# google-research/weatherbench2

Hardware: AMD Instinct MI355X
Metric: grid-point-evals/sec (721x1440x13) (higher is better)
Workload: dtype f32 (elementwise) + f64 (sums); 1 GPU; BASELINE configs[1]: 721x1440x13 f32, deterministic MSE+RMSE+MAE+Bias+ACC, 13 predefined slice regions, running init-time mean; pool_units=48, regions=13, rows_per_chunk=32, step=one wb2_det_suite_step call (K1 + K2 + time accumulate), parallelism=init-time shards x1, 1 all-reduce of [sum,count], launcher=single process

## Files before the change

### weatherbench2_amd/csrc/energy_score.hip

```cpp
#include "ensemble_kernels.hpp"

namespace wb2 {
namespace {

constexpr int kEnergyWaves = 8;
#ifndef WB2_ENERGY_B
#define WB2_ENERGY_B 8
#endif
#ifndef WB2_ENERGY_ROWS
#define WB2_ENERGY_ROWS 4
#endif

template <typename T, int B, bool SKIPNA, bool WF>
__global__ void __launch_bounds__(kEnergyWaves* kWave)
    energy_partials_kernel(const EnsParams p, const int n_block) {
  constexpr int KQ = 2 * B, K = SKIPNA ? 2 * KQ : KQ, NWF = WF ? 2 : 1;
  const int lane = threadIdx.x & (kWave - 1);
  const int wave = __builtin_amdgcn_readfirstlane(threadIdx.x / kWave);
  const unsigned bx = blockIdx.x;
  const long long o = (long long)blockIdx.z * gridDim.y + blockIdx.y;
  const unsigned rest = bx / (unsigned)p.n_chunk;
  const int chunk = (int)(((long long)(bx - rest * (unsigned)p.n_chunk) +
                           (WB2_ROTATE_CHUNKS ? o : 0)) % p.n_chunk);
  const int tile = (int)(rest % (unsigned)p.n_ctile);
// ... 13 lines not shown
  const int colc = active ? col0 : p.n_col - 1;

  double acc[NWF][1][K];
#pragma unroll
  for (int w = 0; w < NWF; ++w)
#pragma unroll
    for (int k = 0; k < K; ++k) acc[w][0][k] = 0.0;

  const long long slab_elems = (long long)p.n_row * p.n_col;
  const T* xrow0 = static_cast<const T*>(p.ens) + es * slab_elems +
                   (long long)m0 * p.member_stride + (long long)row0 * p.n_col;
  const int lane_bytes = colc * (int)sizeof(T);
  const T* tb = static_cast<const T*>(p.truth) + ts * slab_elems +
                (long long)row0 * p.n_col + colc;
  const double* wfp =
      WF ? p.wfield + (long long)row0 * p.n_col + colc : nullptr;
  constexpr int U = WB2_ENERGY_ROWS;
  auto rows = [&](const int r, auto count_tag) {
    constexpr int N = decltype(count_tag)::value;
    T x[N][B + 1], t[N];
    double wr[N], wf[N];
#pragma unroll
    for (int u = 0; u < N; ++u) {
      const long long off = (long long)(r + u) * p.n_col;
      const T* xrow = xrow0 + off;
#pragma unroll
      for (int j = 0; j <= B; ++j)
        x[u][j] = member_load<T, true>(xrow + j * p.member_stride, lane_bytes,
                                       j < nload ? 0x7fffffff : 0);
      t[u] = __builtin_nontemporal_load(tb + off);
      wr[u] = p.w_row[row0 + r + u];
      wf[u] = 1.0;
      if constexpr (WF) wf[u] = wfp[off];
    }
#pragma unroll
    for (int u = 0; u < N; ++u) {
      const bool inside = !WF || wf[u] > 0.0;
      const double w2 = (WF && inside) ? wr[u] * wf[u] : 0.0;
      auto add = [&](int k, T q, bool live) {
        if (!live) return;
        double v = (double)q, c = 1.0;
        if constexpr (SKIPNA) {
          const bool ok = !is_nan(q);
          v = ok ? v : 0.0;
          c = ok ? 1.0 : 0.0;
        }
        acc[0][0][k] = __builtin_fma(wr[u], v, acc[0][0][k]);
        if constexpr (SKIPNA)
          acc[0][0][KQ + k] = __builtin_fma(wr[u], c, acc[0][0][KQ + k]);
        if constexpr (WF) {
          acc[1][0][k] = __builtin_fma(w2, inside ? v : 0.0, acc[1][0][k]);
          if constexpr (SKIPNA)
            acc[1][0][KQ + k] =
                __builtin_fma(w2, inside ? c : 0.0, acc[1][0][KQ + k]);
        }
      };
#pragma unroll
      for (int j = 0; j < B; ++j) {
        const T d = x[u][j] - t[u];
        add(j, d * d, j < nm);
        const T e = x[u][j] - x[u][j + 1];
        add(B + j, e * e, j < np);
      }
    }
  };
  int r = 0;
#pragma clang loop unroll(disable)
  for (; r + U <= nrow; r += U) rows(r, std::integral_constant<int, U>{});
#pragma clang loop unroll(disable)
  for (; r < nrow; ++r) rows(r, std::integral_constant<int, 1>{});
  if (p.w_col) {
    const double wc = p.w_col[colc];
#pragma unroll
    for (int w = 0; w < NWF; ++w)
#pragma unroll
      for (int k = 0; k < K; ++k) acc[w][0][k] *= wc;
  }
  if (!active) {
#pragma unroll
    for (int w = 0; w < NWF; ++w)
#pragma unroll
      for (int k = 0; k < K; ++k) acc[w][0][k] = 0.0;
  }
  fold_tile_to_segs<NWF, 1, K>(
      acc, lane, tile, col0, col0, p.n_col, p.seg_col0, p.seg_eoff, p.n_seg,
      p.n_ts,
      p.partials + ((o * n_block + block) * p.n_chunk + chunk) *
                       (long long)(NWF * p.n_ts * K));
}

constexpr int kEnergyMaxMembers = 1024;
__global__ void __launch_bounds__(kWave)
    energy_finalize_kernel(const double* __restrict__ means, int block,
                           int n_block, int n_member, int skipna, int n_region,
                           long long n_outer, double* __restrict__ out) {
  __shared__ double root[2][kEnergyMaxMembers];
  const long long idx = blockIdx.x;
  const int lane = threadIdx.x;
  const int r = (int)(idx / n_outer);
  const long long o = idx - (long long)r * n_outer;
  const long long n_virtual = n_outer * n_block;
  const long long row = (long long)n_region * n_virtual;
  const double* base = means + (long long)r * n_virtual + o * n_block;
  for (int m = lane; m < n_member; m += kWave) {
    root[0][m] = sqrt(base[(long long)(m % block) * row + m / block]);
    if (m + 1 < n_member)
      root[1][m] = sqrt(base[(long long)(block + m % block) * row + m / block]);
  }
  __syncthreads();
  if (lane != 0) return;
  auto member_mean = [&](const double* v, int count) {
    double s = 0.0, n = 0.0;
    for (int m = 0; m < count; ++m) {
      const bool keep = !(skipna && is_nan(v[m]));
      s += keep ? v[m] : 0.0;
      n += keep ? 1.0 : 0.0;
    }
    return s / n;
  };
  const double skill = member_mean(root[0], n_member);
  const double spread = n_member == 1 ? 0.0 : member_mean(root[1], n_member - 1);
  const long long plane = (long long)n_region * n_outer;
  out[idx] = skill - 0.5 * spread;
  out[plane + idx] = spread;
  out[2 * plane + idx] = skill;
}

template <typename T, int B>
int launch_energy(const EnsParams& p, int n_block, bool skipna, bool wf,
                  hipStream_t stream) {
  const int n_bgrp = (n_block + kEnergyWaves - 1) / kEnergyWaves;
  const int waves = n_block < kEnergyWaves ? n_block : kEnergyWaves;
  const long long gy = p.n_outer < 32768 ? p.n_outer : 32768;
  const long long gz = (p.n_outer + gy - 1) / gy;
  const dim3 grid((unsigned)(p.n_chunk * p.n_ctile * n_bgrp), (unsigned)gy,
                  (unsigned)gz);
  const dim3 blockdim(waves * kWave);
#define WB2_L(S, W)                                                       \
  hipLaunchKernelGGL((energy_partials_kernel<T, B, S, W>), grid, blockdim, 0, \
                     stream, p, n_block)
  if (skipna) {
    if (wf) WB2_L(true, true); else WB2_L(true, false);
  } else {
    if (wf) WB2_L(false, true); else WB2_L(false, false);
  }
#undef WB2_L
  WB2_HIP_OK(hipGetLastError());
  return 0;
}

int energy_block(bool skipna, bool wf) {
  return (skipna && wf) ? 4 : WB2_ENERGY_B;
}

}
}

extern "C" {

int wb2_energy_layout(int32_t n_member, int skipna, int has_wfield,
                      int32_t* block, int32_t* n_block, int32_t* n_slot) {
  using namespace wb2;
  WB2_REQUIRE(n_member >= 1, "n_member=%d", n_member);
  WB2_REQUIRE(block && n_block && n_slot, "null pointer argument");
  const int b = energy_block(skipna != 0, has_wfield != 0);
  *block = b;
  *n_block = (n_member + b - 1) / b;
// ... 89 lines not shown
```

### weatherbench2_amd/csrc/reduce_common.hpp

```cpp
#pragma once

#include "common.hpp"

#include <cstdint>

#ifndef WB2_ROTATE_CHUNKS
#define WB2_ROTATE_CHUNKS 1
#endif

namespace wb2 {

int combine_slots(int mode, int skipna, int k_slots, const double* partials,
                  int64_t n_outer, int32_t n_chunk, int32_t nwf, int32_t n_seg,
                  const int32_t* seg_eoff, int32_t n_ts,
                  const int32_t* band_chunk0, int32_t n_band,
                  const double* coef_band, const double* coef_seg,
                  const int32_t* region_wf, const double* region_wsum,
                  int32_t n_region, double* sums, double* metrics,
                  void* stream);

__device__ __forceinline__ void swap_halves32(double& a, double& b) {
  const unsigned long long ua = __builtin_bit_cast(unsigned long long, a);
  const unsigned long long ub = __builtin_bit_cast(unsigned long long, b);
  const auto lo = __builtin_amdgcn_permlane32_swap(
// ... 7 lines not shown
  const unsigned long long ua = __builtin_bit_cast(unsigned long long, a);
  const unsigned long long ub = __builtin_bit_cast(unsigned long long, b);
  const auto lo = __builtin_amdgcn_permlane16_swap(
      (unsigned)ua, (unsigned)ub, false, false);
  const auto hi = __builtin_amdgcn_permlane16_swap(
      (unsigned)(ua >> 32), (unsigned)(ub >> 32), false, false);
  a = __builtin_bit_cast(double, ((unsigned long long)hi[0] << 32) | lo[0]);
  b = __builtin_bit_cast(double, ((unsigned long long)hi[1] << 32) | lo[1]);
}

template <int CTRL>
__device__ __forceinline__ double dpp_move(double x) {
  const unsigned long long u = __builtin_bit_cast(unsigned long long, x);
  const unsigned lo = (unsigned)__builtin_amdgcn_update_dpp(
      0, (int)(unsigned)u, CTRL, 0xf, 0xf, false);
  const unsigned hi = (unsigned)__builtin_amdgcn_update_dpp(
      0, (int)(unsigned)(u >> 32), CTRL, 0xf, 0xf, false);
  return __builtin_bit_cast(double, ((unsigned long long)hi << 32) | lo);
}

template <int OFF>
__device__ __forceinline__ double allsum_low_bits(double v) {
  static_assert(OFF >= 1 && OFF <= 32, "lane bit");

  if constexpr (OFF >= 32) v += __shfl_xor(v, 32, kWave);
  if constexpr (OFF >= 16) v += __shfl_xor(v, 16, kWave);
  if constexpr (OFF >= 8) v += dpp_move<0x128>(v);
  if constexpr (OFF >= 4) {
    const unsigned long long u = __builtin_bit_cast(unsigned long long, v);
    const unsigned lo = (unsigned)__builtin_amdgcn_ds_swizzle((int)(unsigned)u,
                                                              0x101F);
    const unsigned hi = (unsigned)__builtin_amdgcn_ds_swizzle(
        (int)(unsigned)(u >> 32), 0x101F);
    v += __builtin_bit_cast(double, ((unsigned long long)hi << 32) | lo);
  }
  if constexpr (OFF >= 2) v += dpp_move<0x4E>(v);
  v += dpp_move<0xB1>(v);
  return v;
}

template <int N, int OFF, int NV>
__device__ __forceinline__ void wave_sum_many_step(double (&v)[NV], int lane,
                                                   int& slot, int& real,
                                                   bool& writer) {
  if constexpr (OFF == 0) {
    return;
  } else if constexpr (N == 1) {
    v[0] = allsum_low_bits<OFF>(v[0]);
    writer = writer && (lane & (2 * OFF - 1)) == 0;
  } else {
    constexpr int H = (N + 1) / 2;
    const bool up = (lane & OFF) != 0;
#pragma unroll
    for (int i = 0; i < H; ++i) {
      double lo = v[i];
      double hi = (H + i < N) ? v[H + i] : 0.0;
      if constexpr (OFF == 32) {
        swap_halves32(lo, hi);
        v[i] = lo + hi;
      } else if constexpr (OFF == 16) {
        swap_halves16(lo, hi);
        v[i] = lo + hi;
      } else {
        const double keep = up ? hi : lo, send = up ? lo : hi;
        v[i] = keep + __shfl_xor(send, OFF, kWave);
      }
    }
    slot += up ? H : 0;
    real = up ? (real > H ? real - H : 0) : (real < H ? real : H);
    wave_sum_many_step<H, OFF / 2, NV>(v, lane, slot, real, writer);
  }
}

template <int N>
__device__ __forceinline__ void wave_sum_many(double (&v)[N], int lane,
                                              int& slot, bool& writes) {
  int real = N;
  bool writer = true;
  slot = 0;
  wave_sum_many_step<N, 32, N>(v, lane, slot, real, writer);
  writes = writer && real > 0;
}

template <int NWF, int VEC, int K>
__device__ __forceinline__ void fold_tile_to_segs(
    const double (&acc)[NWF][VEC][K], int lane, int tile, int col0, int own0,
    int n_col, const int* __restrict__ seg_col0, const int* __restrict__ seg_eoff,
    int n_seg, int n_ts, double* __restrict__ out) {
  constexpr int TILE = kWave * VEC;
  const int tile_c0 = tile * TILE;
  const int tile_c1 = min(tile_c0 + TILE, n_col);
  int s_lo = 0;
  while (seg_col0[s_lo + 1] <= tile_c0) ++s_lo;
  int s_hi = s_lo;
  while (s_hi + 1 < n_seg && seg_col0[s_hi + 1] < tile_c1) ++s_hi;
  for (int s = s_lo; s <= s_hi; ++s) {
    const int c0 = seg_col0[s], c1 = seg_col0[s + 1];
    double v[NWF * K];
#pragma unroll
    for (int w = 0; w < NWF; ++w) {
#pragma unroll
      for (int k = 0; k < K; ++k) v[w * K + k] = 0.0;
#pragma unroll
      for (int e = 0; e < VEC; ++e) {
        const bool in_seg = (col0 + e >= max(c0, own0)) && (col0 + e < c1);
#pragma unroll
        for (int k = 0; k < K; ++k)
          v[w * K + k] += in_seg ? acc[w][e][k] : 0.0;
      }
    }
    int slot;
    bool writes;
    wave_sum_many<NWF * K>(v, lane, slot, writes);
    const int e = seg_eoff[s] + tile - c0 / TILE;
    if (writes) {
      const int w = slot / K, k = slot - w * K;
      out[((long long)w * n_ts + e) * K + k] = v[0];
    }
  }
}

}
```

### weatherbench2_amd/csrc/stream_reduce.hip

```cpp

#include "common.hpp"
#include "trace.hpp"
#include "reduce_common.hpp"
#include "gauss_math.hpp"
#include "wb2hip.h"

#include <atomic>
#include <type_traits>

namespace wb2 {
namespace {

constexpr int kMaxIn = 4;

struct StreamParams {
  const void* in[kMaxIn];
  const long long* slab[kMaxIn];
  const double* w_row;
  const double* w_col;
  const void* wfield;
  const double* aux;
  double scalar;
  const int* chunk_row0;
  const int* chunk_nrow;
// ... 193 lines not shown
        x[k] = v[k];
      }
    }
  } else if constexpr (MODE == WB2_MODE_GAUSS) {
    const T mean = in[0], sd = in[1], y = in[2];
    const T nd = (mean - y) / sd;
    const double z = (double)nd;
    double cdf, pdf;
    far = normal_cdf_pdf<ERFCX_FAR>(z, erfcx_lds, cdf, pdf);
    const double crps =
        (double)sd * (z * (2.0 * cdf - 1.0) + 2.0 * pdf - 0.56418958354775628695);
    const T var = sd * sd;
    if constexpr (SKIPNA) {
      const bool okc = !is_nan(crps), okv = !is_nan(var);
      x[0] = okc ? crps : 0.0;
      x[1] = okv ? (double)var : 0.0;
      x[2] = okc ? 1.0 : 0.0;
      x[3] = okv ? 1.0 : 0.0;
    } else {
      x[0] = crps;
      x[1] = (double)var;
    }
  } else {
    T q[PointOps<MODE>::NQ];
    PointOps<MODE>::template elementwise<T>(in, q);
    PointOps<MODE>::template slots<SKIPNA, T>(q, x);
  }
  return far;
}

#ifndef WB2_U_ROWS
#define WB2_U_ROWS 2
#endif
#ifndef WB2_U_ROWS_NARROW
#define WB2_U_ROWS_NARROW 8
#endif
#ifndef WB2_F32_VEC
#define WB2_F32_VEC 4
#endif
#ifndef WB2_F32_VEC_HEAVY
#define WB2_F32_VEC_HEAVY 4
#endif
#ifndef WB2_NT_LOADS
#define WB2_NT_LOADS 1
#endif
#ifndef WB2_GAUSS_GROUP
#define WB2_GAUSS_GROUP 2
#endif
#ifndef WB2_PACK_PAIRS
#define WB2_PACK_PAIRS 1
#endif

#if WB2_NT_LOADS
#define WB2_LOAD(ptr) __builtin_nontemporal_load(ptr)
#else
#define WB2_LOAD(ptr) (*(ptr))
#endif

#define WB2_GLOBAL __attribute__((address_space(1)))

template <typename T, int VEC>
__device__ __forceinline__ void load_vec(const WB2_GLOBAL T* p, T (&v)[VEC]) {
  if constexpr (VEC == 1) {
    v[0] = WB2_LOAD(p);
  } else {
    typedef T V0 __attribute__((ext_vector_type(VEC)));
    typedef V0 V __attribute__((aligned(sizeof(T))));
    const V0 x = WB2_LOAD(reinterpret_cast<const WB2_GLOBAL V*>(p));
#pragma unroll
    for (int e = 0; e < VEC; ++e) v[e] = x[e];
  }
}

template <int VEC, typename FT>
__device__ __forceinline__ void load_wf(const WB2_GLOBAL FT* p,
                                        double (&v)[VEC]) {
  typedef FT V0 __attribute__((ext_vector_type(VEC)));
  typedef V0 V __attribute__((aligned(sizeof(FT))));
  const V0 x = *reinterpret_cast<const WB2_GLOBAL V*>(p);
#pragma unroll
  for (int e = 0; e < VEC; ++e) v[e] = (double)x[e];
}

template <typename T, int VEC, int MODE, bool SKIPNA, bool WF,
          bool SG = false, typename FT = double>
__global__ void __launch_bounds__(512)
    stream_partials_kernel(const StreamParams p) {
  using M = ModeTraits<MODE, SKIPNA>;
  constexpr int NIN = M::NIN, K = M::K, NWF = WF ? 2 : 1;
  constexpr int U = (sizeof(T) * VEC >= 16)
                        ? (NIN >= 4 ? WB2_U_ROWS / 2 : WB2_U_ROWS)
                        : (sizeof(T) * VEC == 8 ? 2 * WB2_U_ROWS
                                                : WB2_U_ROWS_NARROW);
  constexpr int TILE = kWave * VEC;

  const int lane = threadIdx.x & (kWave - 1);
  const int wave = __builtin_amdgcn_readfirstlane(threadIdx.x / kWave);
  const int nwave = blockDim.x / kWave;
  constexpr bool SLAB_FASTEST = WF || MODE == WB2_MODE_SEEPS;
  const unsigned bx = SLAB_FASTEST ? blockIdx.y : blockIdx.x;
  const unsigned tblk = bx / (unsigned)p.n_chunk;
  const long long o =
      SLAB_FASTEST ? (long long)blockIdx.z * gridDim.x + blockIdx.x
                   : (long long)blockIdx.z * gridDim.y + blockIdx.y;
  int chunk = (int)(bx - tblk * (unsigned)p.n_chunk);
  if (!SLAB_FASTEST && WB2_ROTATE_CHUNKS)
    chunk = (int)(((long long)chunk + o) % p.n_chunk);
  const int tile = (int)tblk * nwave + wave;

  const int row0 = p.chunk_row0[chunk];
  const int nrow = p.chunk_nrow[chunk];
  long long slab_idx[NIN];
#pragma unroll
  for (int i = 0; i < NIN; ++i) {
    const long long* tab =
        p.slab[i] ? p.slab[i] : reinterpret_cast<const long long*>(p.chunk_row0);
    const long long v = tab[(p.slab[i] && o < p.n_outer) ? o : 0];
    slab_idx[i] = p.slab[i] ? v : o;
  }
  const int col0 = tile * TILE + lane * VEC;
  const bool active = tile < p.n_ctile && col0 < p.n_col;
  const int colb = (VEC > 1 && col0 + VEC > p.n_col) ? p.n_col - VEC : col0;
  [[maybe_unused]] const double* erfcx_lds = nullptr;
  if constexpr (MODE == WB2_MODE_GAUSS || MODE == WB2_MODE_GAUSS_THR) {
    __shared__ __attribute__((aligned(16))) double erfcx_table[kErfcxDoubles];
    load_erfcx_table(erfcx_table);
    erfcx_lds = erfcx_table;
  }
  if (nrow <= 0 || tile >= p.n_ctile || o >= p.n_outer) return;

  double acc[NWF][VEC][K];
#pragma unroll
  for (int w = 0; w < NWF; ++w)
#pragma unroll
    for (int e = 0; e < VEC; ++e)
#pragma unroll
      for (int k = 0; k < K; ++k) acc[w][e][k] = 0.0;

  if (active) {
    const T* base[NIN];
#pragma unroll
    for (int i = 0; i < NIN; ++i)
      base[i] = reinterpret_cast<const T*>(
                    static_cast<const char*>(p.in[i]) +
                    slab_idx[i] * p.slab_step_bytes) +
                (long long)row0 * p.n_col;
    const FT* wfp =
        WF ? static_cast<const FT*>(p.wfield) + (long long)row0 * p.n_col
           : nullptr;
    const double* wrp = p.w_row + row0;
    unsigned lane_off = (unsigned)colb * (unsigned)sizeof(T);
    unsigned lane_off_wf = (unsigned)colb * (unsigned)sizeof(FT);
    auto at = [&](const T* row) {
      if constexpr (SG) {
        unsigned long long rp = reinterpret_cast<unsigned long long>(row);
        asm volatile("" : "+s"(rp));
        return reinterpret_cast<const WB2_GLOBAL T*>(
            reinterpret_cast<const WB2_GLOBAL char*>(rp) + lane_off);
      } else {
        return reinterpret_cast<const WB2_GLOBAL T*>(
            reinterpret_cast<unsigned long long>(row + colb));
      }
    };
    auto at_wf = [&](const FT* row) {
      if constexpr (SG) {
        unsigned long long rp = reinterpret_cast<unsigned long long>(row);
        asm volatile("" : "+s"(rp));
        return reinterpret_cast<const WB2_GLOBAL FT*>(
            reinterpret_cast<const WB2_GLOBAL char*>(rp) + lane_off_wf);
      } else {
        return reinterpret_cast<const WB2_GLOBAL FT*>(
            reinterpret_cast<unsigned long long>(row + colb));
      }
    };
    auto pin_offsets = [&]() {
      if constexpr (SG) {
        asm volatile("" : "+v"(lane_off));
        if constexpr (WF) asm volatile("" : "+v"(lane_off_wf));
      }
    };

    auto accumulate = [&](int e, const double (&x)[K], double wfe, double wr) {
#pragma unroll
      for (int k = 0; k < K; ++k)
        acc[0][e][k] = __builtin_fma(wr, x[k], acc[0][e][k]);
      if constexpr (WF) {
        const bool inside = wfe > 0.0;
        const unsigned long long keep = inside ? ~0ull : 0x00000000ffffffffull;
        const double w2 = wr * wfe;
        double xs[K];
#pragma unroll
        for (int k = 0; k < K; ++k) {
          if ((MODE == WB2_MODE_DET || MODE == WB2_MODE_DET_ACC) && k == 1) {
            xs[1] = __builtin_fabs(xs[0]);
          } else {
            xs[k] = __builtin_bit_cast(
                double, __builtin_bit_cast(unsigned long long, x[k]) & keep);
          }
          acc[1][e][k] = __builtin_fma(w2, xs[k], acc[1][e][k]);
        }
      }
    };
    constexpr bool POINT_OPS = MODE == WB2_MODE_DET ||
                               MODE == WB2_MODE_DET_ACC ||
                               MODE == WB2_MODE_WIND;
    constexpr bool PAIRS =
        WB2_PACK_PAIRS && POINT_OPS && sizeof(T) == 4 && VEC % 2 == 0;

    auto consume = [&](const T (&v)[NIN][VEC], const double (&wf)[VEC],
                       double wr, const double* auxrow) {
      if constexpr (PAIRS) {
        typedef T V2 __attribute__((ext_vector_type(2)));
        using Ops = PointOps<POINT_OPS ? MODE : WB2_MODE_DET>;
#pragma unroll
        for (int e = 0; e < VEC; e += 2) {
          V2 in2[NIN], q2[Ops::NQ];
#pragma unroll
          for (int i = 0; i < NIN; ++i) {
            in2[i][0] = v[i][e];
            in2[i][1] = v[i][e + 1];
          }
          Ops::template elementwise<V2>(in2, q2);
#pragma unroll
          for (int h = 0; h < 2; ++h) {
            T q[Ops::NQ];
#pragma unroll
            for (int j = 0; j < Ops::NQ; ++j) q[j] = q2[j][h];
            double x[K];
            Ops::template slots<SKIPNA, T>(q, x);
            accumulate(e + h, x, wf[e + h], wr);
          }
        }
      } else if constexpr (MODE == WB2_MODE_GAUSS ||
                           MODE == WB2_MODE_GAUSS_THR) {
        constexpr int G = VEC < WB2_GAUSS_GROUP ? VEC : WB2_GAUSS_GROUP;
#pragma unroll
        for (int e0 = 0; e0 < VEC; e0 += G) {
          double x[G][K];
          bool far[G], any = false;
#pragma unroll
          for (int g = 0; g < G; ++g) {
            T in[NIN];
#pragma unroll
            for (int i = 0; i < NIN; ++i) in[i] = v[i][e0 + g];
            far[g] = eval_slots<MODE, SKIPNA, T>(in, x[g], 0.0, 0.0, erfcx_lds);
            any = any || far[g];
          }
          if (__builtin_amdgcn_ballot_w64(any) != 0) {
#pragma unroll
            for (int g = 0; g < G; ++g) {
              if (far[g]) {
                T in[NIN];
#pragma unroll
                for (int i = 0; i < NIN; ++i) in[i] = v[i][e0 + g];
                eval_slots<MODE, SKIPNA, T, true>(in, x[g], 0.0, 0.0,
                                                  erfcx_lds);
              }
            }
          }
#pragma unroll
          for (int g = 0; g < G; ++g)
            accumulate(e0 + g, x[g], wf[e0 + g], wr);
        }
      } else {
#pragma unroll
        for (int e = 0; e < VEC; ++e) {
          T in[NIN];
#pragma unroll
          for (int i = 0; i < NIN; ++i) in[i] = v[i][e];
          double x[K];
          if constexpr (MODE == WB2_MODE_SEEPS) {
            eval_slots<MODE, SKIPNA, T>(in, x, auxrow[e], p.scalar);
          } else {
            eval_slots<MODE, SKIPNA, T>(in, x);
          }
          accumulate(e, x, wf[e], wr);
        }
      }
    };

    struct Batch {
      T v[U][NIN][VEC];
      double wf[U][VEC];
      double wr[U];
      double ax[U][VEC];
    };
    auto issue = [&](Batch& bt, int r) {
      pin_offsets();
#pragma unroll
      for (int u = 0; u < U; ++u) {
#pragma unroll
        for (int i = 0; i < NIN; ++i)
          load_vec<T, VEC>(at(base[i] + (long long)(r + u) * p.n_col),
                           bt.v[u][i]);
        if constexpr (WF) {
          load_wf<VEC, FT>(at_wf(wfp + (long long)(r + u) * p.n_col), bt.wf[u]);
        } else {
#pragma unroll
          for (int e = 0; e < VEC; ++e) bt.wf[u][e] = 1.0;
        }
        bt.wr[u] = wrp[r + u];
        if constexpr (MODE == WB2_MODE_SEEPS)
          load_wf<VEC, double>(
              reinterpret_cast<const WB2_GLOBAL double*>(
                  reinterpret_cast<unsigned long long>(
                      p.aux + (long long)(row0 + r + u) * p.n_col + colb)),
              bt.ax[u]);
      }
    };
    auto eat = [&](const Batch& bt, int r) {
#pragma unroll
      for (int u = 0; u < U; ++u)
        consume(bt.v[u], bt.wf[u], bt.wr[u],
                MODE == WB2_MODE_SEEPS ? bt.ax[u] : nullptr);
    };
    int r = 0;
#pragma clang loop unroll(disable)
    for (; r + U <= nrow; r += U) {
      Batch bt;
      issue(bt, r);
      __builtin_amdgcn_sched_barrier(0);
      eat(bt, r);
    }
#pragma clang loop unroll(disable)
    for (; r < nrow; ++r) {
      T v[NIN][VEC];
      double wf[VEC];
      pin_offsets();
#pragma unroll
      for (int i = 0; i < NIN; ++i)
        load_vec<T, VEC>(at(base[i] + (long long)r * p.n_col), v[i]);
      if constexpr (WF) {
        load_wf<VEC, FT>(at_wf(wfp + (long long)r * p.n_col), wf);
      } else {
#pragma unroll
        for (int e = 0; e < VEC; ++e) wf[e] = 1.0;
      }
      consume(v, wf, wrp[r],
              MODE == WB2_MODE_SEEPS
                  ? p.aux + (long long)(row0 + r) * p.n_col + colb
                  : nullptr);
    }
    if (p.w_col) {
#pragma unroll
      for (int e = 0; e < VEC; ++e) {
        const double wc = p.w_col[colb + e];
#pragma unroll
        for (int w = 0; w < NWF; ++w)
#pragma unroll
          for (int k = 0; k < K; ++k) acc[w][e][k] *= wc;
      }
    }
  }

  fold_tile_to_segs<NWF, VEC, K>(
      acc, lane, tile, colb, col0, p.n_col, p.seg_col0, p.seg_eoff, p.n_seg,
      p.n_ts,
      p.partials + (o * p.n_chunk + chunk) * (long long)(NWF * p.n_ts * K));
}

struct PairParams {
  double* wind_partials;
  long long first;
  long long n_pair;
};

template <typename T, int VEC, bool ACC, bool SKIPNA, bool WF,
          typename FT = double>
__global__ void __launch_bounds__(128)
    stream_pair_kernel(const StreamParams p, const PairParams pp) {
  constexpr int MODE = ACC ? WB2_MODE_DET_ACC : WB2_MODE_DET;
  using M = ModeTraits<MODE, SKIPNA>;
  using Ops = PointOps<MODE>;
  using MW = ModeTraits<WB2_MODE_WIND, SKIPNA>;
  constexpr int NIN = M::NIN, KD = M::K, KW = MW::K, NWF = WF ? 2 : 1;
  constexpr int U = WB2_U_ROWS;
  constexpr int TILE = kWave * VEC;
  constexpr bool PAIRS = WB2_PACK_PAIRS && sizeof(T) == 4 && VEC % 2 == 0;
  typedef T VT __attribute__((ext_vector_type(VEC)));
  __shared__ VT handoff[2][U][kWave];

  const int lane = threadIdx.x & (kWave - 1);
  const int role = __builtin_amdgcn_readfirstlane(threadIdx.x / kWave);
  const unsigned bx = WF ? blockIdx.y : blockIdx.x;
  const int tile = (int)(bx / (unsigned)p.n_chunk);
  int chunk = (int)(bx - (unsigned)tile * (unsigned)p.n_chunk);
  const long long pair = WF ? (long long)blockIdx.z * gridDim.x + blockIdx.x
                            : (long long)blockIdx.z * gridDim.y + blockIdx.y;
  if (!WF && WB2_ROTATE_CHUNKS)
    chunk = (int)(((long long)chunk + pair) % p.n_chunk);
  const bool live = pair < pp.n_pair;
  const long long o = pp.first + (live ? pair : 0) + role * pp.n_pair;

  const int row0 = p.chunk_row0[chunk];
  const int nrow = p.chunk_nrow[chunk];
  long long slab_idx[NIN];
#pragma unroll
  for (int i = 0; i < NIN; ++i) slab_idx[i] = p.slab[i] ? p.slab[i][o] : o;
  const int col0 = tile * TILE + lane * VEC;
  const int colb = col0 + VEC > p.n_col ? p.n_col - VEC : col0;
  if (nrow <= 0 || !live) return;

  const T* base[NIN];
#pragma unroll
  for (int i = 0; i < NIN; ++i)
    base[i] = reinterpret_cast<const T*>(static_cast<const char*>(p.in[i]) +
                                         slab_idx[i] * p.slab_step_bytes) +
              (long long)row0 * p.n_col;
  const FT* wfp = WF ? static_cast<const FT*>(p.wfield) +
                           (long long)row0 * p.n_col
                     : nullptr;
  const double* wrp = p.w_row + row0;
  auto at = [&](const T* row) {
    return reinterpret_cast<const WB2_GLOBAL T*>(
        reinterpret_cast<unsigned long long>(row + colb));
  };
  auto at_wf = [&](const FT* row) {
    return reinterpret_cast<const WB2_GLOBAL FT*>(
        reinterpret_cast<unsigned long long>(row + colb));
  };

  auto accumulate = [&](auto& acc, auto is_det, int e, const auto& x,
                        double wfe, double wr) {
    constexpr int K = sizeof(x) / sizeof(double);
#pragma unroll
    for (int k = 0; k < K; ++k)
      acc[0][e][k] = __builtin_fma(wr, x[k], acc[0][e][k]);
    if constexpr (WF) {
      const bool inside = wfe > 0.0;
      const unsigned long long keep = inside ? ~0ull : 0x00000000ffffffffull;
      const double w2 = wr * wfe;
      double xs[K];
#pragma unroll
      for (int k = 0; k < K; ++k) {
        if (decltype(is_det)::value && k == 1) {
          xs[1] = __builtin_fabs(xs[0]);
        } else {
          xs[k] = __builtin_bit_cast(
              double, __builtin_bit_cast(unsigned long long, x[k]) & keep);
        }
        acc[1][e][k] = __builtin_fma(w2, xs[k], acc[1][e][k]);
      }
    }
  };
  auto consume = [&](auto wind_c, auto& acc, auto& accw,
                     const T (&v)[NIN][VEC], const double (&wf)[VEC], double wr,
                     T (&sq)[VEC]) {
    constexpr bool WIND = decltype(wind_c)::value;
    auto point = [&](int e, const T (&q)[Ops::NQ]) {
      double x[KD];
      Ops::template slots<SKIPNA, T>(q, x);
      accumulate(acc, std::true_type{}, e, x, wf[e], wr);
      if constexpr (WIND) {
        const T qw[1] = {sq[e] + q[1]};
        double xw[KW];
        PointOps<WB2_MODE_WIND>::template slots<SKIPNA, T>(qw, xw);
        accumulate(accw, std::false_type{}, e, xw, wf[e], wr);
      } else {
        sq[e] = q[1];
      }
    };
    if constexpr (PAIRS) {
      typedef T V2 __attribute__((ext_vector_type(2)));
#pragma unroll
      for (int e = 0; e < VEC; e += 2) {
        V2 in2[NIN], q2[Ops::NQ];
#pragma unroll
        for (int i = 0; i < NIN; ++i) {
          in2[i][0] = v[i][e];
          in2[i][1] = v[i][e + 1];
        }
        Ops::template elementwise<V2>(in2, q2);
#pragma unroll
        for (int h = 0; h < 2; ++h) {
          T q[Ops::NQ];
#pragma unroll
          for (int j = 0; j < Ops::NQ; ++j) q[j] = q2[j][h];
          point(e + h, q);
        }
      }
    } else {
#pragma unroll
      for (int e = 0; e < VEC; ++e) {
        T in[NIN], q[Ops::NQ];
#pragma unroll
        for (int i = 0; i < NIN; ++i) in[i] = v[i][e];
        Ops::template elementwise<T>(in, q);
        point(e, q);
      }
    }
  };
  auto load_row = [&](int r, T (&v)[NIN][VEC], double (&wf)[VEC], double& wr) {
#pragma unroll
    for (int i = 0; i < NIN; ++i)
      load_vec<T, VEC>(at(base[i] + (long long)r * p.n_col), v[i]);
    if constexpr (WF) {
      load_wf<VEC, FT>(at_wf(wfp + (long long)r * p.n_col), wf);
    } else {
#pragma unroll
      for (int e = 0; e < VEC; ++e) wf[e] = 1.0;
    }
    wr = wrp[r];
  };

  double acc[NWF][VEC][KD];
  double accw[NWF][VEC][KW];
#pragma unroll
  for (int w = 0; w < NWF; ++w)
#pragma unroll
    for (int e = 0; e < VEC; ++e) {
#pragma unroll
      for (int k = 0; k < KD; ++k) acc[w][e][k] = 0.0;
#pragma unroll
      for (int k = 0; k < KW; ++k) accw[w][e][k] = 0.0;
    }

  auto batch_u = [&](auto n_c, int r, int buf) {
    constexpr int N = decltype(n_c)::value;
    T v[N][NIN][VEC];
    double wf[N][VEC], wr[N];
#pragma unroll
    for (int u = 0; u < N; ++u) load_row(r + u, v[u], wf[u], wr[u]);
    __builtin_amdgcn_sched_barrier(0);
#pragma unroll
    for (int u = 0; u < N; ++u) {
      T sq[VEC];
      consume(std::false_type{}, acc, accw, v[u], wf[u], wr[u], sq);
      VT out;
#pragma unroll
      for (int e = 0; e < VEC; ++e) out[e] = sq[e];
      handoff[buf][u][lane] = out;
    }
    __syncthreads();
  };
  auto batch_v = [&](auto n_c, int r, int buf) {
    constexpr int N = decltype(n_c)::value;
    T v[N][NIN][VEC];
    double wf[N][VEC], wr[N];
#pragma unroll
    for (int u = 0; u < N; ++u) load_row(r + u, v[u], wf[u], wr[u]);
    __builtin_amdgcn_sched_barrier(0);
    __syncthreads();
#pragma unroll
    for (int u = 0; u < N; ++u) {
      const VT theirs = handoff[buf][u][lane];
      T sq[VEC];
#pragma unroll
      for (int e = 0; e < VEC; ++e) sq[e] = theirs[e];
      consume(std::true_type{}, acc, accw, v[u], wf[u], wr[u], sq);
    }
  };
  int r = 0, it = 0;
  if (role == 0) {
#pragma clang loop unroll(disable)
    for (; r + U <= nrow; r += U, ++it)
      batch_u(std::integral_constant<int, U>{}, r, it & 1);
#pragma clang loop unroll(disable)
    for (; r < nrow; ++r, ++it)
      batch_u(std::integral_constant<int, 1>{}, r, it & 1);
  } else {
#pragma clang loop unroll(disable)
    for (; r + U <= nrow; r += U, ++it)
      batch_v(std::integral_constant<int, U>{}, r, it & 1);
#pragma clang loop unroll(disable)
    for (; r < nrow; ++r, ++it)
      batch_v(std::integral_constant<int, 1>{}, r, it & 1);
  }

  if (p.w_col) {
#pragma unroll
    for (int e = 0; e < VEC; ++e) {
      const double wc = p.w_col[colb + e];
#pragma unroll
      for (int w = 0; w < NWF; ++w) {
#pragma unroll
        for (int k = 0; k < KD; ++k) acc[w][e][k] *= wc;
#pragma unroll
        for (int k = 0; k < KW; ++k) accw[w][e][k] *= wc;
      }
    }
  }
  fold_tile_to_segs<NWF, VEC, KD>(
      acc, lane, tile, colb, col0, p.n_col, p.seg_col0, p.seg_eoff, p.n_seg,
      p.n_ts,
      p.partials + (o * p.n_chunk + chunk) * (long long)(NWF * p.n_ts * KD));
  if (role == 1)
    fold_tile_to_segs<NWF, VEC, KW>(
        accw, lane, tile, colb, col0, p.n_col, p.seg_col0, p.seg_eoff, p.n_seg,
        p.n_ts,
        pp.wind_partials +
            (pair * p.n_chunk + chunk) * (long long)(NWF * p.n_ts * KW));
}

struct CombineParams {
  const double* partials;
  const int* seg_eoff;
  const int* band_chunk0;
  const double* coef_band;
  const double* coef_seg;
  const int* region_wf;
  const double* region_wsum;
  double* sums;
  double* metrics;
  long long n_outer;
  int n_chunk, nwf, n_seg, n_ts, n_band, n_region, K, mode, skipna;
  int group;
};

__device__ __forceinline__ double nan_if_zero(double d) {
  return d != 0.0 ? d : __builtin_nan("");
}

__device__ __forceinline__ void det_combine_body(const CombineParams& p,
                                                 const long long o,
                                                 double* lds) {
  const int K = p.K;
  const int cell = p.nwf * p.n_seg * K;
  double* bandsum = lds;
  double* rsum = lds + p.n_band * cell;
  const int tid = threadIdx.x;
  double* cseg = rsum + p.n_region * K * (1 + p.n_band);
  double* cband = cseg + p.n_region * p.n_seg;
  for (int i = tid; i < p.n_region * p.n_seg; i += blockDim.x)
    cseg[i] = p.coef_seg[i];
  for (int i = tid; i < p.n_region * p.n_band; i += blockDim.x)
    cband[i] = p.coef_band[i];
  const long long chunk_stride = (long long)p.nwf * p.n_ts * K;
  const double* part = p.partials + o * p.n_chunk * chunk_stride;

  if (p.group > 1) {
    const int G = p.group;
    for (int idx = tid; idx < p.n_band * cell * G; idx += blockDim.x) {
      const int ci = idx / G, g = idx - ci * G;
      const int b = ci / cell, j = ci - b * cell;
      const int w = j / (p.n_seg * K), sk = j - w * (p.n_seg * K);
      const int s = sk / K, k = sk - s * K;
      const int e0 = p.seg_eoff[s], ne = p.seg_eoff[s + 1] - e0;
      const int c0 = p.band_chunk0[b], n = (p.band_chunk0[b + 1] - c0) * ne;
      const double* base = part + ((long long)w * p.n_ts) * K + k +
                           c0 * chunk_stride + (long long)e0 * K;
      int c = g / ne, e = g - c * ne;
      const int dq = G / ne, dr = G - dq * ne;
      auto next = [&]() {
        const double* r = base + c * chunk_stride + (long long)e * K;
        c += dq;
        e += dr;
        if (e >= ne) {
          e -= ne;
          ++c;
        }
        return r;
      };
      double v = 0.0;
      int i = g;
      for (; i + 7 * G < n; i += 8 * G) {
        double t[8];
#pragma unroll
        for (int u = 0; u < 8; ++u) t[u] = *next();
#pragma unroll
        for (int u = 0; u < 8; ++u) v += t[u];
      }
      for (; i < n; i += G) v += *next();
      for (int off = G >> 1; off > 0; off >>= 1) v += __shfl_xor(v, off, kWave);
      if (g == 0) bandsum[ci] = v;
    }
  } else
  for (int idx = tid; idx < p.n_band * cell; idx += blockDim.x) {
    const int b = idx / cell, j = idx - b * cell;
    const int w = j / (p.n_seg * K), sk = j - w * (p.n_seg * K);
    const int s = sk / K, k = sk - s * K;
    const int e0 = p.seg_eoff[s], ne = p.seg_eoff[s + 1] - e0;
    const int c0 = p.band_chunk0[b], n = (p.band_chunk0[b + 1] - c0) * ne;
    const double* base = part + ((long long)w * p.n_ts) * K + k;
    const double* q = base + c0 * chunk_stride + (long long)e0 * K;
// ... 1099 lines not shown
```

Measured before the change: 527.7 billion grid-point-evals/s.

## Load segment tables into lanes and pin kernel arguments in scalar registers

Each lane now loads one entry of the column-segment table, and the segment range for a tile comes from ballot/popcount and readlane instead of a scalar search loop over global memory. Kernel parameters, table pointers and slab indices are hoisted and pinned into SGPRs through empty inline asm constraints, which shortens the prologue and epilogue address math. The chunk rotation modulo becomes a conditional subtract. This adds complexity and SGPR pressure, and gives a second code path for more than 63 segments.

Result: no change. 527.4 billion grid-point-evals/s (-0.1%).

```diff
diff --git a/weatherbench2_amd/csrc/energy_score.hip b/weatherbench2_amd/csrc/energy_score.hip
--- a/weatherbench2_amd/csrc/energy_score.hip
+++ b/weatherbench2_amd/csrc/energy_score.hip
@@ -119,7 +119,7 @@
 #pragma unroll
       for (int k = 0; k < K; ++k) acc[w][0][k] = 0.0;
   }
-  fold_tile_to_segs<NWF, 1, K>(
+  fold_tile_by_tables<NWF, 1, K>(
       acc, lane, tile, col0, col0, p.n_col, p.seg_col0, p.seg_eoff, p.n_seg,
       p.n_ts,
       p.partials + ((o * n_block + block) * p.n_chunk + chunk) *
diff --git a/weatherbench2_amd/csrc/reduce_common.hpp b/weatherbench2_amd/csrc/reduce_common.hpp
--- a/weatherbench2_amd/csrc/reduce_common.hpp
+++ b/weatherbench2_amd/csrc/reduce_common.hpp
@@ -113,8 +113,39 @@
   writes = writer && real > 0;
 }
 
+__device__ __forceinline__ int lane_of_full_wave() {
+  return (int)__builtin_amdgcn_mbcnt_hi(~0u, __builtin_amdgcn_mbcnt_lo(~0u, 0u));
+}
+
+template <int NWF, int VEC, int K, typename Entry>
+__device__ __forceinline__ void fold_one_seg(
+    const double (&acc)[NWF][VEC][K], int lane, int col0, int own0, int c0,
+    int c1, int n_ts, double* __restrict__ out, Entry entry) {
+  double v[NWF * K];
+#pragma unroll
+  for (int w = 0; w < NWF; ++w) {
+#pragma unroll
+    for (int k = 0; k < K; ++k) v[w * K + k] = 0.0;
+#pragma unroll
+    for (int e1 = 0; e1 < VEC; ++e1) {
+      const bool in_seg = (col0 + e1 >= max(c0, own0)) && (col0 + e1 < c1);
+#pragma unroll
+      for (int k = 0; k < K; ++k)
+        v[w * K + k] += in_seg ? acc[w][e1][k] : 0.0;
+    }
+  }
+  int slot;
+  bool writes;
+  wave_sum_many<NWF * K>(v, lane, slot, writes);
+  const int e = entry();
+  if (writes) {
+    const int w = slot / K, k = slot - w * K;
+    out[((long long)w * n_ts + e) * K + k] = v[0];
+  }
+}
+
 template <int NWF, int VEC, int K>
-__device__ __forceinline__ void fold_tile_to_segs(
+__device__ __forceinline__ void fold_tile_by_tables(
     const double (&acc)[NWF][VEC][K], int lane, int tile, int col0, int own0,
     int n_col, const int* __restrict__ seg_col0, const int* __restrict__ seg_eoff,
     int n_seg, int n_ts, double* __restrict__ out) {
@@ -151,4 +182,75 @@
   }
 }
 
-}
+struct SegLanes {
+  int col0, eoff;
+};
+constexpr int kSegLaneMax = kWave - 1;
+
+__device__ __forceinline__ SegLanes load_seg_lanes(
+    const int* __restrict__ seg_col0, const int* __restrict__ seg_eoff,
+    int n_seg, int lane) {
+  const int s = min(lane, n_seg);
+  SegLanes sl;
+  sl.col0 = seg_col0[s];
+  sl.eoff = seg_eoff[s];
+  return sl;
+}
+
+template <int NWF, int VEC, int K>
+__device__ __forceinline__ void fold_tile_to_segs(
+    const double (&acc)[NWF][VEC][K], int lane, int tile, int col0, int own0,
+    int n_col, const SegLanes sl, const int* __restrict__ seg_col0,
+    const int* __restrict__ seg_eoff, int n_seg, int n_ts,
+    double* __restrict__ out) {
+  constexpr int TILE = kWave * VEC;
+  const int tile_c0 = tile * TILE;
+  const int tile_c1 = min(tile_c0 + TILE, n_col);
+  const bool by_lane = n_seg <= kSegLaneMax;
+  int s_lo, s_hi;
+  if (by_lane) {
+    s_lo = __builtin_popcountll(
+               __builtin_amdgcn_ballot_w64(sl.col0 <= tile_c0)) - 1;
+    s_hi = __builtin_popcountll(__builtin_amdgcn_ballot_w64(
+               lane < n_seg && sl.col0 < tile_c1)) - 1;
+  } else {
+    s_lo = 0;
+    asm("; wb2-seg-tables-begin" : "+s"(s_lo));
+    while (seg_col0[s_lo + 1] <= tile_c0) ++s_lo;
+    s_hi = s_lo;
+    while (s_hi + 1 < n_seg && seg_col0[s_hi + 1] < tile_c1) ++s_hi;
+    s_lo = __builtin_amdgcn_readfirstlane(s_lo);
+    s_hi = __builtin_amdgcn_readfirstlane(s_hi);
+    asm("; wb2-seg-tables-end" : "+s"(s_lo), "+s"(s_hi));
+  }
+  for (int s = s_lo; s <= s_hi; ++s) {
+    int c0, c1, e0;
+    if (by_lane) {
+      c0 = __builtin_amdgcn_readlane(sl.col0, s);
+      c1 = __builtin_amdgcn_readlane(sl.col0, s + 1);
+      e0 = __builtin_amdgcn_readlane(sl.eoff, s);
+    } else {
+      int at = s;
+      asm("; wb2-seg-tables-begin" : "+s"(at));
+      c0 = __builtin_amdgcn_readfirstlane(seg_col0[at]);
+      c1 = __builtin_amdgcn_readfirstlane(seg_col0[at + 1]);
+      e0 = __builtin_amdgcn_readfirstlane(seg_eoff[at]);
+      asm("; wb2-seg-tables-end" : "+s"(c0), "+s"(c1), "+s"(e0));
+    }
+    fold_one_seg<NWF, VEC, K>(acc, lane, col0, own0, c0, c1, n_ts, out,
+                              [&]() { return e0 + tile - c0 / TILE; });
+  }
+}
+
+template <int NWF, int VEC, int K>
+__device__ __forceinline__ void fold_tile_to_segs(
+    const double (&acc)[NWF][VEC][K], int lane, int tile, int col0, int own0,
+    int n_col, const int* __restrict__ seg_col0, const int* __restrict__ seg_eoff,
+    int n_seg, int n_ts, double* __restrict__ out) {
+  fold_tile_to_segs<NWF, VEC, K>(
+      acc, lane, tile, col0, own0, n_col,
+      load_seg_lanes(seg_col0, seg_eoff, n_seg, lane), seg_col0, seg_eoff,
+      n_seg, n_ts, out);
+}
+
+}
diff --git a/weatherbench2_amd/csrc/stream_reduce.hip b/weatherbench2_amd/csrc/stream_reduce.hip
--- a/weatherbench2_amd/csrc/stream_reduce.hip
+++ b/weatherbench2_amd/csrc/stream_reduce.hip
@@ -299,6 +299,31 @@
   for (int e = 0; e < VEC; ++e) v[e] = (double)x[e];
 }
 
+#define WB2_SGPRS_1(t, a) asm("" : "+s"(t), "+s"(a))
+#define WB2_SGPRS_2(t, a, b) asm("" : "+s"(t), "+s"(a), "+s"(b))
+#define WB2_SGPRS_6(t, a, b, c, d, e, f)                                  \
+  asm("" : "+s"(t), "+s"(a), "+s"(b), "+s"(c), "+s"(d), "+s"(e), "+s"(f))
+#define WB2_SGPRS_8(t, a, b, c, d, e, f, g, h)                            \
+  asm("" : "+s"(t), "+s"(a), "+s"(b), "+s"(c), "+s"(d), "+s"(e), "+s"(f), \
+      "+s"(g), "+s"(h))
+#define WB2_SGPRS_12(t, a, b, c, d, e, f, g, h, i, j, k, l)               \
+  asm("" : "+s"(t), "+s"(a), "+s"(b), "+s"(c), "+s"(d), "+s"(e), "+s"(f), \
+      "+s"(g), "+s"(h), "+s"(i), "+s"(j), "+s"(k), "+s"(l))
+template <typename P>
+__device__ __forceinline__ P* global_ptr(P* q) {
+  return (P*)reinterpret_cast<WB2_GLOBAL P*>(
+      reinterpret_cast<unsigned long long>(q));
+}
+typedef unsigned long long addr_t;
+
+#define WB2_EPILOGUE_ARGS()  \
+  w_col = p.w_col;           \
+  seg_col0 = p.seg_col0;     \
+  seg_eoff = p.seg_eoff;     \
+  partials = p.partials;     \
+  n_seg = p.n_seg;           \
+  n_ts = p.n_ts
+
 template <typename T, int VEC, int MODE, bool SKIPNA, bool WF,
           bool SG = false, typename FT = double>
 __global__ void __launch_bounds__(512)
@@ -315,29 +340,108 @@
   const int wave = __builtin_amdgcn_readfirstlane(threadIdx.x / kWave);
   const int nwave = blockDim.x / kWave;
   constexpr bool SLAB_FASTEST = WF || MODE == WB2_MODE_SEEPS;
-  const unsigned bx = SLAB_FASTEST ? blockIdx.y : blockIdx.x;
-  const unsigned tblk = bx / (unsigned)p.n_chunk;
-  const long long o =
-      SLAB_FASTEST ? (long long)blockIdx.z * gridDim.x + blockIdx.x
-                   : (long long)blockIdx.z * gridDim.y + blockIdx.y;
-  int chunk = (int)(bx - tblk * (unsigned)p.n_chunk);
-  if (!SLAB_FASTEST && WB2_ROTATE_CHUNKS)
-    chunk = (int)(((long long)chunk + o) % p.n_chunk);
-  const int tile = (int)tblk * nwave + wave;
-
-  const int row0 = p.chunk_row0[chunk];
-  const int nrow = p.chunk_nrow[chunk];
-  long long slab_idx[NIN];
-#pragma unroll
-  for (int i = 0; i < NIN; ++i) {
-    const long long* tab =
-        p.slab[i] ? p.slab[i] : reinterpret_cast<const long long*>(p.chunk_row0);
-    const long long v = tab[(p.slab[i] && o < p.n_outer) ? o : 0];
-    slab_idx[i] = p.slab[i] ? v : o;
+  constexpr bool POINT_MODE = MODE == WB2_MODE_DET ||
+                              MODE == WB2_MODE_DET_ACC || MODE == WB2_MODE_WIND;
+  constexpr bool SEG_LANES = POINT_MODE && !SG;
+  constexpr bool SEGS_EARLY = SEG_LANES && !SKIPNA && sizeof(T) * VEC == 16;
+  constexpr bool PHASED = SEG_LANES;
+  const double* w_col;
+  const int *seg_col0, *seg_eoff;
+  double* partials;
+  int n_col = p.n_col, n_seg, n_ts;
+  long long o;
+  int chunk, tile, row0, nrow;
+  long long slab_idx[kMaxIn] = {};
+  SegLanes sl{};
+  if constexpr (!PHASED) {
+    const unsigned bx = SLAB_FASTEST ? blockIdx.y : blockIdx.x;
+    const unsigned tblk = bx / (unsigned)p.n_chunk;
+    o = SLAB_FASTEST ? (long long)blockIdx.z * gridDim.x + blockIdx.x
+                     : (long long)blockIdx.z * gridDim.y + blockIdx.y;
+    chunk = (int)(bx - tblk * (unsigned)p.n_chunk);
+    if (!SLAB_FASTEST && WB2_ROTATE_CHUNKS)
+      chunk = (int)(((long long)chunk + o) % p.n_chunk);
+    tile = (int)tblk * nwave + wave;
+
+    row0 = p.chunk_row0[chunk];
+    nrow = p.chunk_nrow[chunk];
+#pragma unroll
+    for (int i = 0; i < NIN; ++i) {
+      const long long* tab =
+          p.slab[i] ? p.slab[i] : reinterpret_cast<const long long*>(p.chunk_row0);
+      const long long v = tab[(p.slab[i] && o < p.n_outer) ? o : 0];
+      slab_idx[i] = p.slab[i] ? v : o;
+    }
+  } else {
+    WB2_EPILOGUE_ARGS();
+    unsigned n_chunk = (unsigned)p.n_chunk;
+    unsigned grid_xy = SLAB_FASTEST ? gridDim.x : gridDim.y;
+    long long n_outer = p.n_outer;
+    {
+      addr_t in[kMaxIn] = {}, tabs[kMaxIn] = {};
+#pragma unroll
+      for (int i = 0; i < NIN; ++i) {
+        in[i] = (addr_t)p.in[i];
+        tabs[i] = (addr_t)p.slab[i];
+      }
+      addr_t w_row = (addr_t)p.w_row, rows0 = (addr_t)p.chunk_row0,
+             nrows = (addr_t)p.chunk_nrow, wfield = (addr_t)p.wfield,
+             aux = (addr_t)p.aux;
+      long long step = p.slab_step_bytes;
+      long long n_outer_ = p.n_outer;
+      int n_ctile = p.n_ctile;
+      WB2_SGPRS_12(n_col, n_seg, n_ts, n_chunk, grid_xy, n_outer, w_col,
+                   seg_col0, seg_eoff, partials, w_row, rows0, nrows);
+      WB2_SGPRS_12(n_col, in[0], in[1], in[2], in[3], tabs[0], tabs[1], tabs[2],
+                   tabs[3], wfield, aux, step, n_outer_);
+      WB2_SGPRS_1(n_col, n_ctile);
+    }
+    w_col = global_ptr(w_col);
+    seg_col0 = global_ptr(seg_col0);
+    seg_eoff = global_ptr(seg_eoff);
+    partials = global_ptr(partials);
+    const unsigned bx = SLAB_FASTEST ? blockIdx.y : blockIdx.x;
+    const unsigned tblk = bx / n_chunk;
+    o = SLAB_FASTEST ? (long long)blockIdx.z * grid_xy + blockIdx.x
+                     : (long long)blockIdx.z * grid_xy + blockIdx.y;
+    unsigned chunk_u = bx - tblk * n_chunk;
+    if (!SLAB_FASTEST && WB2_ROTATE_CHUNKS) {
+      chunk_u += (unsigned)o % n_chunk;
+      chunk_u -= chunk_u >= n_chunk ? n_chunk : 0u;
+    }
+    chunk = (int)chunk_u;
+    tile = (int)tblk * nwave + wave;
+
+    addr_t tab[kMaxIn] = {};
+    long long slab_at[kMaxIn] = {};
+#pragma unroll
+    for (int i = 0; i < NIN; ++i) {
+      tab[i] = p.slab[i] ? (addr_t)p.slab[i] : (addr_t)p.chunk_row0;
+      slab_at[i] = (p.slab[i] && o < n_outer) ? o : 0;
+    }
+    WB2_SGPRS_8(n_col, tab[0], tab[1], tab[2], tab[3], slab_at[0], slab_at[1],
+                slab_at[2], slab_at[3]);
+    row0 = p.chunk_row0[chunk];
+    nrow = p.chunk_nrow[chunk];
+#pragma unroll
+    for (int i = 0; i < NIN; ++i)
+      slab_idx[i] =
+          reinterpret_cast<const WB2_GLOBAL long long*>(tab[i])[slab_at[i]];
+    if constexpr (SEGS_EARLY) sl = load_seg_lanes(seg_col0, seg_eoff, n_seg, lane);
+    WB2_SGPRS_6(n_col, row0, nrow, slab_idx[0], slab_idx[1], slab_idx[2],
+                slab_idx[3]);
+#pragma unroll
+    for (int i = 0; i < NIN; ++i) slab_idx[i] = p.slab[i] ? slab_idx[i] : o;
+  }
+  double* out = nullptr;
+  if constexpr (PHASED) {
+    out = partials + (o * p.n_chunk + chunk) * (long long)(NWF * n_ts * K);
+    WB2_SGPRS_1(n_col, out);
+    out = global_ptr(out);
   }
   const int col0 = tile * TILE + lane * VEC;
-  const bool active = tile < p.n_ctile && col0 < p.n_col;
-  const int colb = (VEC > 1 && col0 + VEC > p.n_col) ? p.n_col - VEC : col0;
+  const bool active = tile < p.n_ctile && col0 < n_col;
+  const int colb = (VEC > 1 && col0 + VEC > n_col) ? n_col - VEC : col0;
   [[maybe_unused]] const double* erfcx_lds = nullptr;
   if constexpr (MODE == WB2_MODE_GAUSS || MODE == WB2_MODE_GAUSS_THR) {
     __shared__ __attribute__((aligned(16))) double erfcx_table[kErfcxDoubles];
@@ -361,9 +465,9 @@
       base[i] = reinterpret_cast<const T*>(
                     static_cast<const char*>(p.in[i]) +
                     slab_idx[i] * p.slab_step_bytes) +
-                (long long)row0 * p.n_col;
+                (long long)row0 * n_col;
     const FT* wfp =
-        WF ? static_cast<const FT*>(p.wfield) + (long long)row0 * p.n_col
+        WF ? static_cast<const FT*>(p.wfield) + (long long)row0 * n_col
            : nullptr;
     const double* wrp = p.w_row + row0;
     unsigned lane_off = (unsigned)colb * (unsigned)sizeof(T);
@@ -508,10 +612,10 @@
       for (int u = 0; u < U; ++u) {
 #pragma unroll
         for (int i = 0; i < NIN; ++i)
-          load_vec<T, VEC>(at(base[i] + (long long)(r + u) * p.n_col),
+          load_vec<T, VEC>(at(base[i] + (long long)(r + u) * n_col),
                            bt.v[u][i]);
         if constexpr (WF) {
-          load_wf<VEC, FT>(at_wf(wfp + (long long)(r + u) * p.n_col), bt.wf[u]);
+          load_wf<VEC, FT>(at_wf(wfp + (long long)(r + u) * n_col), bt.wf[u]);
         } else {
 #pragma unroll
           for (int e = 0; e < VEC; ++e) bt.wf[u][e] = 1.0;
@@ -521,7 +625,7 @@
           load_wf<VEC, double>(
               reinterpret_cast<const WB2_GLOBAL double*>(
                   reinterpret_cast<unsigned long long>(
-                      p.aux + (long long)(row0 + r + u) * p.n_col + colb)),
+                      p.aux + (long long)(row0 + r + u) * n_col + colb)),
               bt.ax[u]);
       }
     };
@@ -546,22 +650,23 @@
       pin_offsets();
 #pragma unroll
       for (int i = 0; i < NIN; ++i)
-        load_vec<T, VEC>(at(base[i] + (long long)r * p.n_col), v[i]);
+        load_vec<T, VEC>(at(base[i] + (long long)r * n_col), v[i]);
       if constexpr (WF) {
-        load_wf<VEC, FT>(at_wf(wfp + (long long)r * p.n_col), wf);
+        load_wf<VEC, FT>(at_wf(wfp + (long long)r * n_col), wf);
       } else {
 #pragma unroll
         for (int e = 0; e < VEC; ++e) wf[e] = 1.0;
       }
       consume(v, wf, wrp[r],
               MODE == WB2_MODE_SEEPS
-                  ? p.aux + (long long)(row0 + r) * p.n_col + colb
+                  ? p.aux + (long long)(row0 + r) * n_col + colb
                   : nullptr);
     }
-    if (p.w_col) {
+    if constexpr (!PHASED) w_col = p.w_col;
+    if (w_col) {
 #pragma unroll
       for (int e = 0; e < VEC; ++e) {
-        const double wc = p.w_col[colb + e];
+        const double wc = w_col[colb + e];
 #pragma unroll
         for (int w = 0; w < NWF; ++w)
 #pragma unroll
@@ -570,10 +675,23 @@
     }
   }
 
-  fold_tile_to_segs<NWF, VEC, K>(
-      acc, lane, tile, colb, col0, p.n_col, p.seg_col0, p.seg_eoff, p.n_seg,
-      p.n_ts,
-      p.partials + (o * p.n_chunk + chunk) * (long long)(NWF * p.n_ts * K));
+  if constexpr (!PHASED) {
+    WB2_EPILOGUE_ARGS();
+    out = partials + (o * p.n_chunk + chunk) * (long long)(NWF * n_ts * K);
+  }
+  constexpr bool LANE_AGAIN =
+      !POINT_MODE || (MODE == WB2_MODE_DET && SKIPNA && !WF && !SG &&
+                      sizeof(T) * VEC == 16);
+  const int lane_f = LANE_AGAIN ? lane_of_full_wave() : lane;
+  if constexpr (!SEG_LANES) {
+    fold_tile_by_tables<NWF, VEC, K>(acc, lane_f, tile, colb, col0, n_col,
+                                     seg_col0, seg_eoff, n_seg, n_ts, out);
+  } else {
+    if constexpr (!SEGS_EARLY)
+      sl = load_seg_lanes(seg_col0, seg_eoff, n_seg, lane_f);
+    fold_tile_to_segs<NWF, VEC, K>(acc, lane_f, tile, colb, col0, n_col, sl,
+                                   seg_col0, seg_eoff, n_seg, n_ts, out);
+  }
 }
 
 struct PairParams {
@@ -599,23 +717,87 @@
 
   const int lane = threadIdx.x & (kWave - 1);
   const int role = __builtin_amdgcn_readfirstlane(threadIdx.x / kWave);
+  constexpr bool SEGS_EARLY = !SKIPNA && sizeof(T) * VEC == 16;
+  const double* w_col;
+  const int *seg_col0, *seg_eoff;
+  double* partials;
+  int n_col = p.n_col, n_seg, n_ts;
+  long long pair;
+  bool live;
+  long long o;
+  int chunk, tile, row0, nrow;
+  long long slab_idx[kMaxIn] = {};
+  SegLanes sl{};
+  WB2_EPILOGUE_ARGS();
+  unsigned n_chunk = (unsigned)p.n_chunk;
+  unsigned grid_xy = WF ? gridDim.x : gridDim.y;
+  long long n_pair = pp.n_pair;
+  {
+    addr_t in[kMaxIn] = {}, tabs[kMaxIn] = {};
+#pragma unroll
+    for (int i = 0; i < NIN; ++i) {
+      in[i] = (addr_t)p.in[i];
+      tabs[i] = (addr_t)p.slab[i];
+    }
+    addr_t w_row = (addr_t)p.w_row, rows0 = (addr_t)p.chunk_row0,
+           nrows = (addr_t)p.chunk_nrow, wfield = (addr_t)p.wfield,
+           aux = (addr_t)p.aux;
+    long long step = p.slab_step_bytes;
+    addr_t wind = (addr_t)pp.wind_partials;
+    long long first = pp.first;
+    WB2_SGPRS_12(n_col, n_seg, n_ts, n_chunk, grid_xy, n_pair, w_col,
+                 seg_col0, seg_eoff, partials, w_row, rows0, nrows);
+    WB2_SGPRS_12(n_col, in[0], in[1], in[2], in[3], tabs[0], tabs[1], tabs[2],
+                 tabs[3], wfield, aux, step, wind);
+    WB2_SGPRS_1(n_col, first);
+  }
+  w_col = global_ptr(w_col);
+  seg_col0 = global_ptr(seg_col0);
+  seg_eoff = global_ptr(seg_eoff);
+  partials = global_ptr(partials);
   const unsigned bx = WF ? blockIdx.y : blockIdx.x;
-  const int tile = (int)(bx / (unsigned)p.n_chunk);
-  int chunk = (int)(bx - (unsigned)tile * (unsigned)p.n_chunk);
-  const long long pair = WF ? (long long)blockIdx.z * gridDim.x + blockIdx.x
-                            : (long long)blockIdx.z * gridDim.y + blockIdx.y;
-  if (!WF && WB2_ROTATE_CHUNKS)
-    chunk = (int)(((long long)chunk + pair) % p.n_chunk);
-  const bool live = pair < pp.n_pair;
-  const long long o = pp.first + (live ? pair : 0) + role * pp.n_pair;
-
-  const int row0 = p.chunk_row0[chunk];
-  const int nrow = p.chunk_nrow[chunk];
-  long long slab_idx[NIN];
-#pragma unroll
-  for (int i = 0; i < NIN; ++i) slab_idx[i] = p.slab[i] ? p.slab[i][o] : o;
+  tile = (int)(bx / n_chunk);
+  pair = WF ? (long long)blockIdx.z * grid_xy + blockIdx.x
+                            : (long long)blockIdx.z * grid_xy + blockIdx.y;
+  unsigned chunk_u = bx - (unsigned)tile * n_chunk;
+  if (!WF && WB2_ROTATE_CHUNKS) {
+    chunk_u += (unsigned)pair % n_chunk;
+    chunk_u -= chunk_u >= n_chunk ? n_chunk : 0u;
+  }
+  chunk = (int)chunk_u;
+  live = pair < n_pair;
+  o = pp.first + (live ? pair : 0) + role * n_pair;
+
+  addr_t tab[kMaxIn] = {};
+  long long slab_at[kMaxIn] = {};
+#pragma unroll
+  for (int i = 0; i < NIN; ++i) {
+    tab[i] = p.slab[i] ? (addr_t)p.slab[i] : (addr_t)p.chunk_row0;
+    slab_at[i] = p.slab[i] ? o : 0;
+  }
+  WB2_SGPRS_8(n_col, tab[0], tab[1], tab[2], tab[3], slab_at[0], slab_at[1],
+              slab_at[2], slab_at[3]);
+  row0 = p.chunk_row0[chunk];
+  nrow = p.chunk_nrow[chunk];
+#pragma unroll
+  for (int i = 0; i < NIN; ++i)
+    slab_idx[i] =
+        reinterpret_cast<const WB2_GLOBAL long long*>(tab[i])[slab_at[i]];
+  if constexpr (SEGS_EARLY) sl = load_seg_lanes(seg_col0, seg_eoff, n_seg, lane);
+  WB2_SGPRS_6(n_col, row0, nrow, slab_idx[0], slab_idx[1], slab_idx[2],
+              slab_idx[3]);
+#pragma unroll
+  for (int i = 0; i < NIN; ++i) slab_idx[i] = p.slab[i] ? slab_idx[i] : o;
+
+  double* out =
+      partials + (o * p.n_chunk + chunk) * (long long)(NWF * n_ts * KD);
+  double* out_wind = pp.wind_partials +
+                     (pair * p.n_chunk + chunk) * (long long)(NWF * n_ts * KW);
+  WB2_SGPRS_2(n_col, out, out_wind);
+  out = global_ptr(out);
+  out_wind = global_ptr(out_wind);
   const int col0 = tile * TILE + lane * VEC;
-  const int colb = col0 + VEC > p.n_col ? p.n_col - VEC : col0;
+  const int colb = col0 + VEC > n_col ? n_col - VEC : col0;
   if (nrow <= 0 || !live) return;
 
   const T* base[NIN];
@@ -623,9 +805,9 @@
   for (int i = 0; i < NIN; ++i)
     base[i] = reinterpret_cast<const T*>(static_cast<const char*>(p.in[i]) +
                                          slab_idx[i] * p.slab_step_bytes) +
-              (long long)row0 * p.n_col;
+              (long long)row0 * n_col;
   const FT* wfp = WF ? static_cast<const FT*>(p.wfield) +
-                           (long long)row0 * p.n_col
+                           (long long)row0 * n_col
                      : nullptr;
   const double* wrp = p.w_row + row0;
   auto at = [&](const T* row) {
@@ -710,9 +892,9 @@
   auto load_row = [&](int r, T (&v)[NIN][VEC], double (&wf)[VEC], double& wr) {
 #pragma unroll
     for (int i = 0; i < NIN; ++i)
-      load_vec<T, VEC>(at(base[i] + (long long)r * p.n_col), v[i]);
+      load_vec<T, VEC>(at(base[i] + (long long)r * n_col), v[i]);
     if constexpr (WF) {
-      load_wf<VEC, FT>(at_wf(wfp + (long long)r * p.n_col), wf);
+      load_wf<VEC, FT>(at_wf(wfp + (long long)r * n_col), wf);
     } else {
 #pragma unroll
       for (int e = 0; e < VEC; ++e) wf[e] = 1.0;
@@ -784,10 +966,10 @@
       batch_v(std::integral_constant<int, 1>{}, r, it & 1);
   }
 
-  if (p.w_col) {
+  if (w_col) {
 #pragma unroll
     for (int e = 0; e < VEC; ++e) {
-      const double wc = p.w_col[colb + e];
+      const double wc = w_col[colb + e];
 #pragma unroll
       for (int w = 0; w < NWF; ++w) {
 #pragma unroll
@@ -797,16 +979,13 @@
       }
     }
   }
-  fold_tile_to_segs<NWF, VEC, KD>(
-      acc, lane, tile, colb, col0, p.n_col, p.seg_col0, p.seg_eoff, p.n_seg,
-      p.n_ts,
-      p.partials + (o * p.n_chunk + chunk) * (long long)(NWF * p.n_ts * KD));
+  if constexpr (!SEGS_EARLY)
+    sl = load_seg_lanes(seg_col0, seg_eoff, n_seg, lane);
+  fold_tile_to_segs<NWF, VEC, KD>(acc, lane, tile, colb, col0, n_col, sl,
+                                  seg_col0, seg_eoff, n_seg, n_ts, out);
   if (role == 1)
-    fold_tile_to_segs<NWF, VEC, KW>(
-        accw, lane, tile, colb, col0, p.n_col, p.seg_col0, p.seg_eoff, p.n_seg,
-        p.n_ts,
-        pp.wind_partials +
-            (pair * p.n_chunk + chunk) * (long long)(NWF * p.n_ts * KW));
+    fold_tile_to_segs<NWF, VEC, KW>(accw, lane, tile, colb, col0, n_col, sl,
+                                    seg_col0, seg_eoff, n_seg, n_ts, out_wind);
 }
 
 struct CombineParams {
```
